# deadskull7/One-Stop-for-COVID-19-Infection-and-Lung-Segmentation-plus-Classification

Hardware: AMD Instinct MI355X
Metric: CT images/sec (fwd+bwd) U-Net 512x512x1 bs16 (higher is better)
Workload: dtype f32 storage / accumulate / parameters; conv products as a two-term fp16 split (3 fp16 MFMAs per multiply, ~2^-22 per product; --algo 2 = strict fp32); 1 GPU; U-Net infection seg (task1 graph T1:853-916), 512x512x1, batch 16/GPU, fp32, fwd+loss+bwd+Keras-Adam; BASELINE.json configs[1]; storage=fp32, global_batch=16, parallelism=dp1, deterministic=False, bn_fold=2

## Files before the change

include/unet_hip.h:

```cpp
#ifndef UNET_HIP_H
#define UNET_HIP_H
#include <stddef.h>
#include <stdint.h>

#ifdef __cplusplus
extern "C" {
#endif

#define UNET_ABI_VERSION 16

typedef struct unet_ctx unet_ctx;
typedef struct unet_model unet_model;
typedef uint16_t unet_bf16;
enum { UNET_DTYPE_F32 = 0, UNET_DTYPE_BF16 = 1 };

enum { UNET_OK = 0, UNET_E_ARG = -1, UNET_E_HIP = -2, UNET_E_SHAPE = -3, UNET_E_STATE = -4, UNET_E_NODEV = -5 };

enum { UNET_ALGO_AUTO = 0, UNET_ALGO_NAIVE = 1, UNET_ALGO_MFMA = 2 };

int32_t unet_abi_version(void);
int32_t unet_ctx_create(int32_t device_id, unet_ctx** out);
void unet_ctx_destroy(unet_ctx* ctx);
const char* unet_last_error(const unet_ctx* ctx);
int32_t unet_ctx_set_profiling(unet_ctx* ctx, int32_t on);
enum { UNET_OPT_RELU_BITS = 1, UNET_OPT_BN_FOLD = 2, UNET_OPT_ENC_BN_FUSED = 3, UNET_OPT_BN_CONCAT_ANALYTIC = 4, UNET_OPT_BN_FUSE_STATS = 5, UNET_OPT_DETERMINISTIC = 6,
       UNET_OPT_HEAD_FUSED = 7, UNET_OPT_SKIP_RAW = 8, UNET_OPT_POOL_SUMS_FUSED = 9, UNET_OPT_HEAD_BWD_FUSED = 10, UNET_OPT_CONV_PP = 13, UNET_OPT_ENC_TAIL_DGRAD = 14,
       UNET_OPT_WGRAD_EARLY_SPLIT = 15 };
int32_t unet_ctx_set_option(unet_ctx* ctx, int32_t option, int32_t value);
int32_t unet_ctx_get_option(unet_ctx* ctx, int32_t option);

enum { UNET_ACT_NONE = 0, UNET_ACT_RELU = 1, UNET_ACT_ELU = 2 };
enum { UNET_MASK_NONE = 0, UNET_MASK_RELU = 1, UNET_MASK_ELU = 2, UNET_MASK_ELU_DROP = 3, UNET_MASK_RELU_BITS = 9  };

size_t unet_conv3x3_w_ws_floats(int32_t cin, int32_t cout);
int32_t unet_conv3x3_pick_algo(int32_t algo, int32_t wd, int32_t cin, int32_t cout);
double unet_conv3x3_exec_ratio(int32_t algo, int32_t h, int32_t wd, int32_t cin, int32_t cout);
double unet_conv3x3_wgrad_exec_ratio(int32_t algo, int32_t h, int32_t wd, int32_t cin, int32_t cout);
int32_t unet_request_bn_stats(unet_ctx*, int32_t c);
int32_t unet_relu_bits_supported(int32_t algo, int32_t h, int32_t wd, int32_t cin, int32_t cout);
size_t unet_relu_bits_bytes(int32_t n, int32_t h, int32_t wd, int32_t c);
int32_t unet_request_relu_bits(unet_ctx*, void* bits);
int32_t unet_allow_k_slices(unet_ctx*);
int32_t unet_ctx_max_kernel_scratch_bytes(unet_ctx*);
int32_t unet_conv3x3_fwd(unet_ctx*, const float* x, const float* w, const float* bias, float* y,
                         int32_t n, int32_t h, int32_t wd, int32_t cin, int32_t cout,
                         int32_t act, float drop_rate, uint64_t drop_seed, int32_t algo, float* w_ws, void* stream);
int32_t unet_conv3x3_fwd_ld(unet_ctx*, const float* x, const float* w, const float* bias, float* y, int32_t ldy,
                            int32_t n, int32_t h, int32_t wd, int32_t cin, int32_t cout, int32_t act, int32_t algo, float* w_ws, void* stream);
int32_t unet_conv3x3_bwd_data(unet_ctx*, const float* dy, const float* w, const float* mask_src,
                              int32_t mask_mode, float mask_rate, uint64_t mask_seed,
// ... 8 lines not shown
                                        int32_t cin, int32_t cout, int32_t algo, void* stream);
int32_t unet_conv3x3_bnfold_bwd_data(unet_ctx*, const float* dy, const float* w, const float* bnp, const double* bn_bwd_sums, double count, const float* x,
                                     int32_t x_channels, int32_t mask_mode, float mask_rate, uint64_t mask_seed, float* dx, float* wt_ws, float* coef,
                                     int32_t n, int32_t h, int32_t wd, int32_t cin, int32_t cout, int32_t algo, void* stream);
int32_t unet_conv3x3_bnfold_bwd_data_enc_tail(unet_ctx*, const float* dy, const float* w, const float* bnp, const double* bn_bwd_sums, double count, const float* x, int32_t ldx,
                                              const float* enc_bnp, const double* enc_sums, double enc_count, const float* skip_k1, const float* dy_pooled, float rate,
                                              uint64_t seed, float* dx, float* wt_ws, float* coef, int32_t n, int32_t h, int32_t wd, int32_t c, int32_t algo, void* stream);
size_t unet_conv3x3_bwd_weights_ws_bytes(int32_t n, int32_t h, int32_t wd, int32_t cin, int32_t cout);
int32_t unet_conv3x3_bwd_weights(unet_ctx*, const float* x, const float* dy, float* dw, float* db,
                                 void* ws, size_t ws_bytes, int32_t n, int32_t h, int32_t wd,
                                 int32_t cin, int32_t cout, int32_t algo, void* stream);

int32_t unet_convT2x2_fwd(unet_ctx*, const float* x, const float* w, const float* bias, float* y,
                          int32_t ldy, int32_t n, int32_t h, int32_t wd, int32_t cin, int32_t cout,
                          int32_t algo, void* stream);
int32_t unet_convT2x2_bwd_data(unet_ctx*, const float* dy, int32_t lddy, const float* w,
                               const float* relu_src, float* dx, int32_t n, int32_t h, int32_t wd,
                               int32_t cin, int32_t cout, int32_t algo, void* stream);
size_t unet_convT2x2_bwd_weights_ws_bytes(int32_t n, int32_t h, int32_t wd, int32_t cin, int32_t cout);
int32_t unet_convT2x2_bwd_weights(unet_ctx*, const float* x, const float* dy, int32_t lddy,
                                  float* dw, float* db, void* ws, size_t ws_bytes, int32_t n,
                                  int32_t h, int32_t wd, int32_t cin, int32_t cout, int32_t algo,
                                  void* stream);

int32_t unet_bn_stats(unet_ctx*, const float* x, int32_t ldx, double* sums, int64_t pixels,
                      int32_t c, void* stream);
int32_t unet_bn_stats_concat(unet_ctx*, const float* x_up, int32_t ldx, const double* src_sums, double src_count, const float* src_gamma,
                             const float* src_beta, double* sums, int64_t pixels, int32_t c_up, int32_t c_skip, void* stream);
int32_t unet_bn_finalize_train(unet_ctx*, const double* sums, double count, const float* gamma,
                               const float* beta, float* moving_mean, float* moving_var,
                               float* bnp, int32_t c, void* stream);
int32_t unet_bn_finalize_infer(unet_ctx*, const float* gamma, const float* beta,
                               const float* moving_mean, const float* moving_var, float* bnp,
                               int32_t c, void* stream);
int32_t unet_bn_apply(unet_ctx*, const float* x, int32_t ldx, const float* bnp, float* y,
                      int32_t ldy, int64_t pixels, int32_t c, void* stream);
int32_t unet_bn_bwd_stats(unet_ctx*, const float* dy, int32_t lddy, const float* x, int32_t ldx,
                          const float* bnp, double* sums, int64_t pixels, int32_t c, void* stream);
int32_t unet_bn_bwd_param_grads(unet_ctx*, const double* sums, float* dgamma, float* dbeta,
                                int32_t c, void* stream);
int32_t unet_bn_bwd_apply(unet_ctx*, const float* dy, int32_t lddy, const float* x, int32_t ldx,
                          const float* bnp, const double* sums, double count, int32_t mask_mode,
                          float mask_rate, uint64_t mask_seed, float* dx, int32_t lddx, int64_t pixels,
                          int32_t c, void* stream);

int32_t unet_maxpool2x2_dropout_fwd(unet_ctx*, const float* x, int32_t ldx, float* y, int32_t n,
// ... 399 lines not shown
```

one-stop-for-covid-19-infection-and-lung-segmentation-plus-classification_amd/_lib.py:

```python
from __future__ import annotations

import ctypes as C
import os

_HERE = os.path.dirname(os.path.abspath(__file__))
LIB_PATH = os.environ.get("COVIDSEG_AMD_LIB") or os.path.join(_HERE, "libunet_hip.so")
ABI_VERSION = 16
COMM_HANDLE_BYTES, COMM_MAX_WORLD, COMM_MAX_DOUBLES = 64, 8, 2048

ALGO_AUTO, ALGO_NAIVE, ALGO_MFMA = 0, 1, 2
OPTIONS = {"relu_bits": 1, "bn_fold": 2, "enc_bn_fused": 3, "bn_concat_analytic": 4, "bn_fuse_stats": 5, "deterministic": 6, "head_fused": 7, "skip_raw": 8, "pool_sums_fused": 9, "head_bwd_fused": 10, "conv_pp": 13, "enc_tail_dgrad": 14, "wgrad_early_split": 15}
ARCH_UNET, ARCH_UNETPP, ARCH_CLASSIFIER = 0, 1, 2
LOSSES = {"bce_dice_loss": 0, "binary_crossentropy": 1, "dice_loss": 2, "tversky_loss": 3, "weighted_bce_dice_loss": 4}
DTYPE_F32, DTYPE_BF16 = 0, 1
ACT_NONE, ACT_RELU, ACT_ELU = 0, 1, 2
MORPH_OPS = {"dilate": 0, "erode": 1, "open": 2, "close": 3}
MORPH_MAX_ITERATIONS = 64
INTENSITY_MAX_EDGES = 63
JOINT_HIST_MAX_K, JOINT_HIST_MAX_BINS = 16, 64
SMOOTH_MAX_RADIUS = 32
PAIRS_CHUNK, PAIRS_LDS_SLOTS = 4096, 1024
PAIRS_MIN_CAPACITY, PAIRS_MAX_CAPACITY = 16, 2 ** 30
TRACK_CLS_NONE, TRACK_CLS_RESOLVED, TRACK_CLS_SHRINKAGE, TRACK_CLS_BOTH, TRACK_CLS_GROWTH, TRACK_CLS_NEW = 0, 1, 2, 3, 4, 5
TEXTURE_MAX_LEVELS, TEXTURE_MAX_DISTANCE, TEXTURE_LDS_COUNTERS = 64, 4, 8192
TEXTURE_MAX_RUN = 2 ** 15
ZONE_MAX_PARTS, ZONE_MAX_SHELLS, ZONE_MAX_BINS = 8, 4, 1024
RANK_MAX_RADIUS = 2
FILTER_MODES = {"nearest": 0, "constant": 1, "reflect": 2}
GEODESIC_MAX_STEP = 65534
MASK_NONE, MASK_RELU, MASK_ELU, MASK_ELU_DROP = 0, 1, 2, 3
PROG_FWD_TRAIN, PROG_BWD, PROG_FWD_INFER = 0, 1, 2
SYNC_BN_FWD, SYNC_LOSS, SYNC_BN_BWD, SYNC_GRAD_BUCKET = 0, 1, 2, 3

f32p = C.POINTER(C.c_float)
# ... 37 lines not shown
    "unet_relu_bits_supported": (i32, [i32, i32, i32, i32, i32]),
    "unet_relu_bits_bytes": (sz, [i32, i32, i32, i32]),
    "unet_request_relu_bits": (i32, [vp, vp]),
    "unet_allow_k_slices": (i32, [vp]),
    "unet_ctx_max_kernel_scratch_bytes": (i32, [vp]),
    "unet_conv3x3_fwd": (i32, [vp, vp, vp, vp, vp, i32, i32, i32, i32, i32, i32, f32, u64, i32, vp, vp]),
    "unet_conv3x3_fwd_ld": (i32, [vp, vp, vp, vp, vp, i32, i32, i32, i32, i32, i32, i32, i32, vp, vp]),
    "unet_conv3x3_bwd_data": (i32, [vp, vp, vp, vp, i32, f32, u64, vp, vp, i32, i32, i32, i32, i32, i32, vp]),
    "unet_conv3x3_bwd_weights_ws_bytes": (sz, [i32, i32, i32, i32, i32]),
    "unet_conv3x3_bwd_weights": (i32, [vp, vp, vp, vp, vp, vp, sz, i32, i32, i32, i32, i32, i32, vp]),
    "unet_convT2x2_fwd": (i32, [vp, vp, vp, vp, vp, i32, i32, i32, i32, i32, i32, i32, vp]),
    "unet_convT2x2_bwd_data": (i32, [vp, vp, i32, vp, vp, vp, i32, i32, i32, i32, i32, i32, vp]),
    "unet_convT2x2_bwd_weights_ws_bytes": (sz, [i32, i32, i32, i32, i32]),
    "unet_convT2x2_bwd_weights": (i32, [vp, vp, vp, i32, vp, vp, vp, sz, i32, i32, i32, i32, i32, i32, vp]),
    "unet_cast_f32_to_bf16": (i32, [vp, vp, vp, i64, vp]),
    "unet_cast_bf16_to_f32": (i32, [vp, vp, vp, i64, vp]),
    "unet_conv3x3_fwd_bf16": (i32, [vp, vp, vp, vp, vp, i32, i32, i32, i32, i32, i32, f32, u64, vp, vp]),
    "unet_conv3x3_first_fwd_bf16": (i32, [vp, vp, vp, vp, vp, i32, i32, i32, i32, i32, f32, u64, vp]),
    "unet_conv3x3_bwd_data_bf16": (i32, [vp, vp, vp, vp, i32, f32, u64, vp, vp, i32, i32, i32, i32, i32, vp]),
    "unet_conv3x3_bwd_weights_ws_bytes_bf16": (sz, [i32, i32, i32, i32, i32]),
    "unet_conv3x3_bwd_weights_bf16": (i32, [vp, vp, vp, vp, vp, vp, sz, i32, i32, i32, i32, i32, vp]),
    "unet_conv3x3_first_bwd_weights_bf16": (i32, [vp, vp, vp, vp, vp, vp, sz, i32, i32, i32, i32, vp]),
    "unet_convT2x2_fwd_bf16": (i32, [vp, vp, vp, vp, vp, i32, i32, i32, i32, i32, i32, vp, vp]),
    "unet_convT2x2_bwd_data_bf16": (i32, [vp, vp, i32, vp, vp, vp, i32, i32, i32, i32, i32, vp, vp]),
    "unet_convT2x2_bwd_weights_ws_bytes_bf16": (sz, [i32, i32, i32, i32, i32]),
    "unet_convT2x2_bwd_weights_bf16": (i32, [vp, vp, vp, i32, vp, vp, vp, sz, i32, i32, i32, i32, i32, vp]),
    "unet_bn_stats": (i32, [vp, vp, i32, vp, i64, i32, vp]),
    "unet_bn_stats_bf16": (i32, [vp, vp, i32, vp, i64, i32, vp]),
    "unet_conv3x3_bnfold_supported": (i32, [i32, i32, i32, i32, i32]),
    "unet_conv3x3_bnfold_ws_floats": (sz, [i32, i32, i32]),
    "unet_conv3x3_bnfold_fwd": (i32, [vp, vp, vp, vp, vp, vp, i32, i32, i32, i32, i32, i32, i32, vp, vp]),
    "unet_conv3x3_bnfold_bwd_weights": (i32, [vp, vp, vp, vp, vp, vp, vp, vp, vp, sz, vp, i32, i32, i32, i32, i32, i32, vp]),
    "unet_conv3x3_bnfold_bwd_data": (i32, [vp, vp, vp, vp, vp, f64, vp, i32, i32, f32, u64, vp, vp, vp, i32, i32, i32, i32, i32, i32, vp]),
    "unet_conv3x3_bnfold_bwd_data_enc_tail": (i32, [vp, vp, vp, vp, vp, f64, vp, i32, vp, vp, f64, vp, vp, f32, u64, vp, vp, vp, i32, i32, i32, i32, i32, vp]),
    "unet_bn_stats_concat": (i32, [vp, vp, i32, vp, f64, vp, vp, vp, i64, i32, i32, vp]),
    "unet_bn_stats_concat_bf16": (i32, [vp, vp, i32, vp, f64, vp, vp, vp, i64, i32, i32, vp]),
    "unet_bn_finalize_train": (i32, [vp, vp, f64, vp, vp, vp, vp, vp, i32, vp]),
    "unet_bn_finalize_infer": (i32, [vp, vp, vp, vp, vp, vp, i32, vp]),
    "unet_bn_apply": (i32, [vp, vp, i32, vp, vp, i32, i64, i32, vp]),
    "unet_bn_apply_bf16": (i32, [vp, vp, i32, vp, vp, i32, i64, i32, vp]),
    "unet_bn_bwd_stats": (i32, [vp, vp, i32, vp, i32, vp, vp, i64, i32, vp]),
    "unet_bn_bwd_stats_bf16": (i32, [vp, vp, i32, vp, i32, vp, vp, i64, i32, vp]),
    "unet_bn_bwd_param_grads": (i32, [vp, vp, vp, vp, i32, vp]),
    "unet_bn_bwd_apply": (i32, [vp, vp, i32, vp, i32, vp, vp, f64, i32, f32, u64, vp, i32, i64, i32, vp]),
    "unet_bn_bwd_apply_bf16": (i32, [vp, vp, i32, vp, i32, vp, vp, f64, i32, f32, u64, vp, i32, i64, i32, vp]),
    "unet_maxpool2x2_dropout_fwd": (i32, [vp, vp, i32, vp, i32, i32, i32, i32, f32, u64, vp]),
# ... 241 lines not shown
```

one-stop-for-covid-19-infection-and-lung-segmentation-plus-classification_amd/csrc/common.h:

```cpp
#pragma once
#include <hip/hip_runtime.h>
#include <stdint.h>
#include <stdio.h>
#include <set>
#include <string>

#include "../../include/unet_hip.h"

constexpr int UNET_BN_SLOTS = 64, UNET_BN_SLOTS_DET = 1024, UNET_BN_SLOT_DOUBLES = 2048;
struct unet_loss_sel { int32_t kind = UNET_LOSS_BCE_DICE; float alpha = 0.5f, beta = 0.5f; };
inline bool unet_loss_sel_ok(const unet_loss_sel& ls, const float* wm = nullptr, bool need_map = true) {
  if (ls.kind < UNET_LOSS_BCE_DICE || ls.kind > UNET_LOSS_WEIGHTED_BCE_DICE) return false;
  if (ls.kind == UNET_LOSS_TVERSKY && !(ls.alpha > 0.0f && ls.beta > 0.0f && ls.alpha < 1e30f && ls.beta < 1e30f)) return false;
  return !need_map || (ls.kind == UNET_LOSS_WEIGHTED_BCE_DICE) == (wm != nullptr);
}
constexpr int UNET_HEAD_SUMS = 100;
struct unet_ctx {
  int device = 0;
  int num_cu = 256;
  int profiling = 0;
  int opt_relu_bits = 1;
  int opt_bn_fold = 2;
  int opt_enc_bn_fused = 1;
  int opt_bn_concat_analytic = 1;
  int opt_bn_fuse_stats = 1;
  int opt_pool_sums_fused = 1;
  int opt_skip_raw = 1;
  int opt_head_fused = 1;
  int opt_head_bwd_fused = 1;
  int opt_enc_tail_dgrad = 1;
  int opt_wgrad_early_split = 0;
  int opt_conv_pp = 1;
  int opt_deterministic = 0;
  double* bn_slots = nullptr;
  int bn_nslots() const { return opt_deterministic ? UNET_BN_SLOTS_DET : UNET_BN_SLOTS; }
  void* convt_img = nullptr;
  size_t convt_img_bytes = 0;
  int k_slices_ok = 0;
  void* splitk_ws = nullptr;
  size_t splitk_ws_bytes = 0;
  int stats_req_c = 0;
  const void* stats_in_slots = nullptr;
  int stats_in_slots_c = 0;
  bool stats_in_slots_xs = false;
  unsigned long long* signs_req = nullptr;
  const void* signs_done = nullptr;
  std::set<const void*> big_lds_kernels;
  std::set<const void*> noted_kernels;
  int max_scratch_bytes = 0;
  std::string err;
};

#define UNET_FAIL(ctx, code, ...)                         \
  do {                                                    \
// ... 326 lines not shown
```

one-stop-for-covid-19-infection-and-lung-segmentation-plus-classification_amd/csrc/model.hip:

```cpp
#include <algorithm>
#include <functional>
#include <map>
#include <set>
#include <string>
#include <vector>

#include "common.h"

extern "C" {

int32_t unet_abi_version(void) { return UNET_ABI_VERSION; }

int32_t unet_ctx_create(int32_t device_id, unet_ctx** out) {
  if (!out) return UNET_E_ARG;
  *out = nullptr;
  int ndev = 0;
  if (hipGetDeviceCount(&ndev) != hipSuccess || ndev <= 0 || device_id < 0 || device_id >= ndev) return UNET_E_NODEV;
  hipDeviceProp_t prop;
  if (hipGetDeviceProperties(&prop, device_id) != hipSuccess) return UNET_E_NODEV;
  if (std::string(prop.gcnArchName).rfind("gfx950", 0) != 0) return UNET_E_NODEV;
  unet_ctx* c = new unet_ctx();
  c->device = device_id;
  c->num_cu = prop.multiProcessorCount;
  const size_t sb = sizeof(double) * UNET_BN_SLOTS_DET * UNET_BN_SLOT_DOUBLES;
// ... 14 lines not shown
  if (ctx && ctx->bn_slots) (void)hipFree(ctx->bn_slots);
  if (ctx && ctx->convt_img) (void)hipFree(ctx->convt_img);
  if (ctx && ctx->splitk_ws) (void)hipFree(ctx->splitk_ws);
  delete ctx;
}
const char* unet_last_error(const unet_ctx* ctx) { return ctx ? ctx->err.c_str() : "null ctx"; }
int32_t unet_ctx_set_profiling(unet_ctx* ctx, int32_t on) { if (!ctx) return UNET_E_ARG; ctx->profiling = on; return UNET_OK; }

static int* ctx_option(unet_ctx* ctx, int32_t option) {
  switch (option) {
    case UNET_OPT_RELU_BITS: return &ctx->opt_relu_bits;
    case UNET_OPT_BN_FOLD: return &ctx->opt_bn_fold;
    case UNET_OPT_ENC_BN_FUSED: return &ctx->opt_enc_bn_fused;
    case UNET_OPT_BN_CONCAT_ANALYTIC: return &ctx->opt_bn_concat_analytic;
    case UNET_OPT_BN_FUSE_STATS: return &ctx->opt_bn_fuse_stats;
    case UNET_OPT_DETERMINISTIC: return &ctx->opt_deterministic;
    case UNET_OPT_HEAD_FUSED: return &ctx->opt_head_fused;
    case UNET_OPT_SKIP_RAW: return &ctx->opt_skip_raw;
    case UNET_OPT_POOL_SUMS_FUSED: return &ctx->opt_pool_sums_fused;
    case UNET_OPT_HEAD_BWD_FUSED: return &ctx->opt_head_bwd_fused;
    case UNET_OPT_CONV_PP: return &ctx->opt_conv_pp;
    case UNET_OPT_ENC_TAIL_DGRAD: return &ctx->opt_enc_tail_dgrad;
    case UNET_OPT_WGRAD_EARLY_SPLIT: return &ctx->opt_wgrad_early_split;
    default: return nullptr;
  }
}
int32_t unet_ctx_set_option(unet_ctx* ctx, int32_t option, int32_t value) {
  if (!ctx) return UNET_E_ARG;
  int* p = ctx_option(ctx, option);
  const int hi = option == UNET_OPT_BN_FOLD ? 3 : (option == UNET_OPT_CONV_PP || option == UNET_OPT_ENC_TAIL_DGRAD) ? 2 : 1;
  if (!p || value < 0 || value > hi) UNET_FAIL(ctx, UNET_E_ARG, "ctx_set_option: option %d value %d", option, value);
  *p = value;
  return UNET_OK;
}
int32_t unet_ctx_get_option(unet_ctx* ctx, int32_t option) {
  if (!ctx) return UNET_E_ARG;
  const int* p = ctx_option(ctx, option);
  if (!p) UNET_FAIL(ctx, UNET_E_ARG, "ctx_get_option: unknown option %d", option);
  return *p;
}

}

static bool use_mfma(int algo, int cin, int cout) {
  if (algo == UNET_ALGO_NAIVE) return false;
  return mfma_conv3x3_supported(cin, cout);
}
static bool use_h2(int algo, int cin, int cout, const void* uws) { return uws && h2_conv3x3_selected(algo, cin, cout); }

static int32_t conv3x3_fwd_dispatch(unet_ctx* ctx, const float* x, const float* w, const float* bias, const float* mask, int mask_mode,
                                    float* y, int n, int h, int wd, int cin, int cout, int act, float rate, uint64_t seed, int algo,
                                    hipStream_t s, float* uws = nullptr, int flip = 0, const float* prepared = nullptr, int ldy = 0) {
  if (ldy && ldy != cout && !(use_h2(algo, cin, cout, uws) && prepared)) UNET_FAIL(ctx, UNET_E_STATE, "conv3x3: a strided output (ldy %d) exists on the h2 kernels with a prepared image only", ldy);
// ... 601 lines not shown
    } else {
      m->grad[nm] = mk(cv, b.n, b.h, b.w, b.c);
    }
  }
  size_t wgb = 0;
  int S2 = m->H, T2 = m->W;
  (void)S2; (void)T2;
  {
    int s = m->H, t = m->W, idx = 0;
    for (auto& l : m->layers) {
      (void)idx;
      if (l.kind != 0) continue;
      int lvl;
      if (l.name == "c5a" || l.name == "c5b") lvl = 4;
      else { int k = l.name[1] - '0'; lvl = (k <= 4) ? k - 1 : 9 - k; }
      int hs = s >> lvl, ts = t >> lvl;
      wgb = std::max(wgb, m->dt ? unet_conv3x3_bwd_weights_ws_bytes_bf16(m->N, hs, ts, l.cin, l.cout) : unet_conv3x3_bwd_weights_ws_bytes(m->N, hs, ts, l.cin, l.cout));
    }
    for (auto& l : m->layers) {
      if (l.kind != 1) continue;
      int k = l.name[1] - '0';
      int lvl = 10 - k;
      wgb = std::max(wgb, m->dt ? bf16_convT_wgrad_ws_bytes(m->N, s >> lvl, t >> lvl, l.cin, l.cout) : unet_convT2x2_bwd_weights_ws_bytes(m->N, s >> lvl, t >> lvl, l.cin, l.cout));
    }
  }
  m->wgrad_ws_bytes = wgb;
  m->off_wgrad_ws = cv.take((wgb + 3) / 4);
  m->ws_floats_train = cv.cur;
}

double nel(const Buf& b) { return (double)b.n * b.h * b.w * b.c; }

#define ADD_OP(vec, nm, fl, by, ...)                          \
  do {                                                        \
    Op _o; _o.name = (nm); _o.flops = (fl); _o.bytes = (by);  \
    _o.run = [=](hipStream_t s) -> int32_t __VA_ARGS__;       \
    (vec).push_back(std::move(_o));                           \
  } while (0)

void arm_bn_statistics(unet_model* m) {
  auto& F = m->prog[UNET_PROG_FWD_TRAIN];
  unet_ctx* ctx = m->ctx;
  for (size_t i = 1; i < F.size(); ++i) {
    if (F[i].name.rfind("bn_stats:", 0) != 0 || F[i - 1].name.rfind("conv3x3_fwd:", 0) != 0) continue;
    const std::string bn = F[i].name.substr(9);
    const auto g = m->tinfo.find(bn + "/gamma");
// ... 402 lines not shown
      const TInfo a = m->tinfo.at(first), b = m->tinfo.at(last_tensor);
      SY.push_back({(int)BW.size() - 1, 3, false, (size_t)a.off * 4, b.off + b.count - a.off});
    };
    if (!dt && m->skip_raw && ctx->opt_enc_bn_fused && ctx->opt_enc_tail_dgrad)
      for (int k = 1; k <= 4; ++k) {
        const std::string bnn = "bn" + std::to_string(k), dca = "c" + std::to_string(10 - k) + "a", cb = "c" + std::to_string(k) + "b";
        const Buf xb = m->act.at(bnn), cg = m->grad.at(cb);
        if (m->fold_c_off.count(dca) && m->skip_k1_off.count(bnn) && m->wprep_b.count(dca) && cg.ld == xb.c && m->act.at(dca).c == xb.c &&
            h2_enc_tail_dgrad_selected(ctx, algo, xb.n, xb.h, xb.w, xb.c, ctx->opt_enc_tail_dgrad == 2))
          m->enc_tail_dgrad.insert(bnn);
      }
    bool enc_split = false;
    const int dec[4] = {256, 128, 64, 32};
    for (int k = 9; k >= 6; --k) {
      int c = dec[k - 6]; std::string ks = std::to_string(k);
      std::string prev = (k == 6) ? "c5b" : "c" + std::to_string(k - 1) + "b";
      int cprev = (k == 6) ? 512 : dec[k - 7];
      conv_bwd("c" + ks + "b", "c" + ks + "a", c, c, true, true, "", m->fold_c_off.count("c" + ks + "a") != 0);
      conv_bwd("c" + ks + "a", "bn" + ks, 2 * c, c, true, false, m->fold_off.count("c" + ks + "a") ? "cat" + ks : "");
      flush_def();
      if (!m->fold_c_off.count("c" + ks + "a")) bn_bwd("bn" + ks, "bn" + ks, "cat" + ks, "cat" + ks, 2 * c, 0, m->fold_off.count("c" + ks + "a") != 0);
      const Buf ib = m->act.at(prev), ug = m->grad.at("u" + ks);
      const std::string un = "u" + ks;
      ADD_OP(BW, "convT_wgrad:" + un, 2.0 * 4 * cprev * c * nel(ib) / ib.c, eb * (nel(ib) + nel(ug)), {
        if (dt) return k_convT_bf16_wgrad(ctx, CBF(m->Av(prev)), CBF(m->Dv(un)), ug.ld, m->G(un + "/kernel"), m->G(un + "/bias"), m->wsf(m->off_wgrad_ws), m->wgrad_ws_bytes, ib.n, ib.h,
                                          ib.w, cprev, c, s);
        return unet_convT2x2_bwd_weights(ctx, m->A(prev), m->D(un), ug.ld, m->G(un + "/kernel"), m->G(un + "/bias"), m->wsf(m->off_wgrad_ws), m->wgrad_ws_bytes,
                                         ib.n, ib.h, ib.w, cprev, c, algo, s);
      });
      ADD_OP(BW, "convT_dgrad:" + un, 2.0 * 4 * cprev * c * nel(ib) / ib.c, eb * (2 * nel(ib) + nel(ug)), {
        if (dt) return k_convT_bf16_dgrad(ctx, CBF(m->Dv(un)), ug.ld, m->P(un + "/kernel"), CBF(m->Av(prev)), WBF(m->Dv(prev)), ib.n, ib.h, ib.w, cprev, c, WBF(static_cast<void*>(m->wsf(m->off_wt))), s);
        const auto so = m->sign_off.find(prev);
        const auto pb = m->wprep_b.find(un);
        const void* img = pb == m->wprep_b.end() ? nullptr : m->wsf(pb->second);
        if (so != m->sign_off.end()) return k_convT_h2_dgrad(ctx, m->D(un), ug.ld, m->P(un + "/kernel"), m->wsf(so->second), m->D(prev), ib.n, ib.h, ib.w, cprev, c, s, 1, img);
        if (img) return k_convT_h2_dgrad(ctx, m->D(un), ug.ld, m->P(un + "/kernel"), m->A(prev), m->D(prev), ib.n, ib.h, ib.w, cprev, c, s, 0, img);
        return unet_convT2x2_bwd_data(ctx, m->D(un), ug.ld, m->P(un + "/kernel"), m->A(prev), m->D(prev), ib.n, ib.h, ib.w, cprev, c, algo, s);
      });
      if (k == 7) bucket("u7/kernel", "out/bias");
      if (k == 6) bucket("u6/kernel", "c6b/bias");
    }
    conv_bwd("c5b", "c5a", 512, 512, true, true);
    conv_bwd("c5a", "p4", 256, 512, true, false, "", ctx->opt_enc_bn_fused != 0);
    if (!ctx->opt_enc_bn_fused) bucket("c5a/kernel", "c5b/bias");
    for (int k = 4; k >= 1; --k) {
      int c = ENC[k - 1]; std::string ks = std::to_string(k);
      const Buf xb = m->act.at("bn" + ks), gb = m->grad.at("bn" + ks);
      const std::string bnn = "bn" + ks, pn = "p" + ks;
      const size_t so = m->bn_bsum_off.at(bnn);
      if (ctx->opt_enc_bn_fused) {
        const std::string dn = "bn" + std::to_string(10 - k), cb = "c" + ks + "b";
        const size_t sod = m->bn_bsum_off.at(dn), bod = m->bnp_off.at(dn), bo = m->bnp_off.at(bnn);
        const Buf cbuf = m->act.at(cb), cg = m->grad.at(cb);
// ... 1008 lines not shown
```

Measured before the change: 1078 images/sec.

## Fuse transposed-conv weight and data gradients into one MFMA kernel

Adds a new HIP kernel that computes the convT2x2 weight gradient and data gradient together in one pass. It loads the upsampled gradient tile into LDS once as split fp16 hi/lo pairs and reuses it for both the wgrad and dgrad MFMAs, applying the ReLU mask inline. The decoder backward graph uses it by default for the shapes it supports (cout 32 or 64). The goal is to avoid reading dU and the activations twice across two kernels and to drop a launch, at the cost of higher register and LDS pressure plus a partial-sum reduction workspace.

```diff
diff --git a/include/unet_hip.h b/include/unet_hip.h
--- a/include/unet_hip.h
+++ b/include/unet_hip.h
@@ -25,7 +25,7 @@
 int32_t unet_ctx_set_profiling(unet_ctx* ctx, int32_t on);
 enum { UNET_OPT_RELU_BITS = 1, UNET_OPT_BN_FOLD = 2, UNET_OPT_ENC_BN_FUSED = 3, UNET_OPT_BN_CONCAT_ANALYTIC = 4, UNET_OPT_BN_FUSE_STATS = 5, UNET_OPT_DETERMINISTIC = 6,
        UNET_OPT_HEAD_FUSED = 7, UNET_OPT_SKIP_RAW = 8, UNET_OPT_POOL_SUMS_FUSED = 9, UNET_OPT_HEAD_BWD_FUSED = 10, UNET_OPT_CONV_PP = 13, UNET_OPT_ENC_TAIL_DGRAD = 14,
-       UNET_OPT_WGRAD_EARLY_SPLIT = 15 };
+       UNET_OPT_WGRAD_EARLY_SPLIT = 15, UNET_OPT_CONVT_BWD_FUSED = 16 };
 int32_t unet_ctx_set_option(unet_ctx* ctx, int32_t option, int32_t value);
 int32_t unet_ctx_get_option(unet_ctx* ctx, int32_t option);
 
@@ -80,6 +80,11 @@
                                   float* dw, float* db, void* ws, size_t ws_bytes, int32_t n,
                                   int32_t h, int32_t wd, int32_t cin, int32_t cout, int32_t algo,
                                   void* stream);
+
+int32_t unet_convT2x2_bwd_fused_selected(unet_ctx*, int32_t n, int32_t h, int32_t wd, int32_t cin, int32_t cout, int32_t force);
+size_t unet_convT2x2_bwd_fused_ws_bytes(int32_t n, int32_t h, int32_t wd, int32_t cin, int32_t cout);
+int32_t unet_convT2x2_bwd_fused(unet_ctx*, const float* x, const float* dy, int32_t lddy, const float* kernel, const void* mask, int32_t mask_is_bits, float* dx, float* dw,
+                                float* db, void* ws, size_t ws_bytes, int32_t n, int32_t h, int32_t wd, int32_t cin, int32_t cout, void* stream);
 
 int32_t unet_bn_stats(unet_ctx*, const float* x, int32_t ldx, double* sums, int64_t pixels,
                       int32_t c, void* stream);
diff --git a/one-stop-for-covid-19-infection-and-lung-segmentation-plus-classification_amd/_lib.py b/one-stop-for-covid-19-infection-and-lung-segmentation-plus-classification_amd/_lib.py
--- a/one-stop-for-covid-19-infection-and-lung-segmentation-plus-classification_amd/_lib.py
+++ b/one-stop-for-covid-19-infection-and-lung-segmentation-plus-classification_amd/_lib.py
@@ -9,7 +9,7 @@
 COMM_HANDLE_BYTES, COMM_MAX_WORLD, COMM_MAX_DOUBLES = 64, 8, 2048
 
 ALGO_AUTO, ALGO_NAIVE, ALGO_MFMA = 0, 1, 2
-OPTIONS = {"relu_bits": 1, "bn_fold": 2, "enc_bn_fused": 3, "bn_concat_analytic": 4, "bn_fuse_stats": 5, "deterministic": 6, "head_fused": 7, "skip_raw": 8, "pool_sums_fused": 9, "head_bwd_fused": 10, "conv_pp": 13, "enc_tail_dgrad": 14, "wgrad_early_split": 15}
+OPTIONS = {"relu_bits": 1, "bn_fold": 2, "enc_bn_fused": 3, "bn_concat_analytic": 4, "bn_fuse_stats": 5, "deterministic": 6, "head_fused": 7, "skip_raw": 8, "pool_sums_fused": 9, "head_bwd_fused": 10, "conv_pp": 13, "enc_tail_dgrad": 14, "wgrad_early_split": 15, "convT_bwd_fused": 16}
 ARCH_UNET, ARCH_UNETPP, ARCH_CLASSIFIER = 0, 1, 2
 LOSSES = {"bce_dice_loss": 0, "binary_crossentropy": 1, "dice_loss": 2, "tversky_loss": 3, "weighted_bce_dice_loss": 4}
 DTYPE_F32, DTYPE_BF16 = 0, 1
@@ -93,6 +93,9 @@
     "unet_conv3x3_bwd_weights_bf16": (i32, [vp, vp, vp, vp, vp, vp, sz, i32, i32, i32, i32, i32, vp]),
     "unet_conv3x3_first_bwd_weights_bf16": (i32, [vp, vp, vp, vp, vp, vp, sz, i32, i32, i32, i32, vp]),
     "unet_convT2x2_fwd_bf16": (i32, [vp, vp, vp, vp, vp, i32, i32, i32, i32, i32, i32, vp, vp]),
+    "unet_convT2x2_bwd_fused_selected": (i32, [vp, i32, i32, i32, i32, i32, i32]),
+    "unet_convT2x2_bwd_fused_ws_bytes": (sz, [i32, i32, i32, i32, i32]),
+    "unet_convT2x2_bwd_fused": (i32, [vp, vp, vp, i32, vp, vp, i32, vp, vp, vp, vp, sz, i32, i32, i32, i32, i32, vp]),
     "unet_convT2x2_bwd_data_bf16": (i32, [vp, vp, i32, vp, vp, vp, i32, i32, i32, i32, i32, vp, vp]),
     "unet_convT2x2_bwd_weights_ws_bytes_bf16": (sz, [i32, i32, i32, i32, i32]),
     "unet_convT2x2_bwd_weights_bf16": (i32, [vp, vp, vp, i32, vp, vp, vp, sz, i32, i32, i32, i32, i32, vp]),
diff --git a/one-stop-for-covid-19-infection-and-lung-segmentation-plus-classification_amd/csrc/common.h b/one-stop-for-covid-19-infection-and-lung-segmentation-plus-classification_amd/csrc/common.h
--- a/one-stop-for-covid-19-infection-and-lung-segmentation-plus-classification_amd/csrc/common.h
+++ b/one-stop-for-covid-19-infection-and-lung-segmentation-plus-classification_amd/csrc/common.h
@@ -30,6 +30,7 @@
   int opt_head_bwd_fused = 1;
   int opt_enc_tail_dgrad = 1;
   int opt_wgrad_early_split = 0;
+  int opt_convT_bwd_fused = 1;
   int opt_conv_pp = 1;
   int opt_deterministic = 0;
   double* bn_slots = nullptr;
diff --git a/one-stop-for-covid-19-infection-and-lung-segmentation-plus-classification_amd/csrc/kernels_convT_bwd.hip b/one-stop-for-covid-19-infection-and-lung-segmentation-plus-classification_amd/csrc/kernels_convT_bwd.hip
--- /dev/null
+++ b/one-stop-for-covid-19-infection-and-lung-segmentation-plus-classification_amd/csrc/kernels_convT_bwd.hip
@@ -0,0 +1,388 @@
+#include <stdlib.h>
+
+#include <algorithm>
+
+#include "common.h"
+
+namespace {
+
+typedef _Float16 f16x8 __attribute__((ext_vector_type(8)));
+typedef short s16x4 __attribute__((ext_vector_type(4)));
+typedef short s16x8 __attribute__((ext_vector_type(8)));
+typedef float f32x4 __attribute__((ext_vector_type(4)));
+typedef unet_f32x16 f32x16;
+
+__device__ __forceinline__ float pow2f(int e) { return __uint_as_float((unsigned)(e + 127) << 23); }
+
+__device__ __forceinline__ f16x8 lds_tr_frag(const char* p0, const char* p1) {
+  typedef __attribute__((address_space(3))) s16x4 lds_s16x4;
+  const s16x4 a = __builtin_amdgcn_ds_read_tr16_b64_v4i16((lds_s16x4*)(p0));
+  const s16x4 b = __builtin_amdgcn_ds_read_tr16_b64_v4i16((lds_s16x4*)(p1));
+  const s16x8 v = __builtin_shufflevector(a, b, 0, 1, 2, 3, 4, 5, 6, 7);
+  return __builtin_bit_cast(f16x8, v);
+}
+
+enum { CTB_MASK_NONE = 0, CTB_MASK_F32 = 1, CTB_MASK_BITS = 2 };
+
+template <int NA>
+__global__ __launch_bounds__(256, 2) void convT_bwd_kernel(const float* __restrict__ A, int ldA, const float* __restrict__ B, const float* __restrict__ Wk, const void* __restrict__ mask,
+                                                           int mask_mode, float* __restrict__ dx, float* __restrict__ part, int N, int H, int W, int CA, int CB, int tiles_b, int strips,
+                                                           int rows_per_chunk, int chunks_per_strip, int nsplit, long long pstride, int units, int upb) {
+  static_assert(NA == 1 || NA == 2, "32 or 64 dU channels");
+  constexpr int R = 1;
+  constexpr int TAPS = 4, AROWS = 2 * R, KP = NA == 1 ? 2 : 1;
+  constexpr int PPL = 32 * 64 + 64, ROWB = 2 * PPL;
+  constexpr int ASUB = AROWS * ROWB, BSUB = R * 32 * 64;
+  constexpr int STAGE1 = NA * ASUB + 2 * BSUB;
+  constexpr int RED = KP > 1 ? 2 * TAPS * 16 * 64 * 4 : 0;
+  constexpr int STAGE = 2 * STAGE1;
+  __shared__ __attribute__((aligned(16))) char smem[STAGE > RED ? STAGE : RED];
+  __shared__ float s_bs[4][64];
+  __shared__ float s_amax[2][4];
+  char* const s_a = smem; char* const s_b = smem + NA * ASUB;
+  const int tid = threadIdx.x, lane = tid & 63, l31 = lane & 31, hi = lane >> 5, l15 = lane & 15, g4 = lane >> 4;
+  const int wave = __builtin_amdgcn_readfirstlane(tid >> 6);
+  const int kp = wave % KP, wb = (wave / KP) % 2, wa = wave / (KP * 2);
+  const int sq = blockIdx.x >> 3;
+  const int tb = sq % tiles_b, split = (sq / tiles_b) * 8 + (blockIdx.x & 7);
+  if (split >= nsplit) return;
+  const int b0 = tb * 64;
+  const int chunk = split % chunks_per_strip; const int ublk = split / chunks_per_strip;
+  const int ya = chunk * rows_per_chunk;
+  const int yb = ya + rows_per_chunk < H ? ya + rows_per_chunk : H;
+  const int HA = 2 * H, WAI = 2 * W;
+
+  f16x8 wfh[TAPS * NA], wfm[TAPS * NA];
+  float unw;
+  {
+    float wv[TAPS * NA][8];
+    float mw = 0.f;
+    const float* wp = Wk + (long long)(g4 * 8) * CB + b0 + wave * 16 + l15;
+#pragma unroll
+    for (int k = 0; k < TAPS * NA; ++k)
+#pragma unroll
+      for (int j = 0; j < 8; ++j) { wv[k][j] = wp[(long long)(k * 32 + j) * CB]; mw = fmaxf(mw, fabsf(wv[k][j])); }
+    mw = wave_max_nonneg(mw);
+    const int ebw = __builtin_amdgcn_readfirstlane((int)((__float_as_uint(mw) >> 23) & 0xFF));
+    const int e_w = ebw >= 11 ? 138 - ebw : 120;
+    const float sw = pow2f(e_w);
+    unw = pow2f(max(-e_w, -126));
+#pragma unroll
+    for (int k = 0; k < TAPS * NA; ++k) {
+      unet_u32x4 h, m;
+#pragma unroll
+      for (int j = 0; j < 4; ++j) { unsigned hh, mm; split2_scaled(wv[k][2 * j], wv[k][2 * j + 1], sw, hh, mm); h[j] = hh; m[j] = mm; }
+      wfh[k] = __builtin_bit_cast(f16x8, h); wfm[k] = __builtin_bit_cast(f16x8, m);
+    }
+  }
+
+  f32x16 acc[TAPS];
+#pragma unroll
+  for (int t = 0; t < TAPS; ++t)
+#pragma unroll
+    for (int r = 0; r < 16; ++r) acc[t][r] = 0.0f;
+  float bsum = 0.0f;
+  int e_a = 120, e_b = 120;
+
+  const int tr_px = (g4 >> 1) * 8 + (l15 >> 2), tr_ch = ((g4 & 1) * 16 + (l15 & 3) * 4) * 2;
+  const char* const pa = s_a + wa * ASUB + tr_ch;
+  const char* const pb = s_b + wb * BSUB + tr_ch;
+  const char* const pd = s_a + l15 * 64 + g4 * 16;
+  const int cq = b0 + wave * 16 + g4 * 4;
+
+  const int u1 = (ublk + 1) * upb < units ? (ublk + 1) * upb : units;
+  for (int unit = ublk * upb; unit < u1; ++unit) {
+    const int cs = unit % strips, n = unit / strips;
+    const int x0 = cs * 32;
+    const __amdgpu_buffer_rsrc_t rs_a = make_rsrc(A + (long long)n * HA * WAI * ldA, (long long)HA * WAI * ldA * 4);
+    const __amdgpu_buffer_rsrc_t rs_b = make_rsrc(B + (long long)n * H * W * CB, (long long)H * W * CB * 4);
+    const int q8 = tid & 7, pc = tid >> 3;
+    int abase_t[NA][2], bbase_t[2];
+#pragma unroll
+    for (int sub = 0; sub < NA; ++sub)
+#pragma unroll
+      for (int half = 0; half < 2; ++half) {
+        const int gx = 2 * x0 + half * 32 + pc;
+        abase_t[sub][half] = gx < WAI ? (gx * ldA + sub * 32 + q8 * 4) * 4 : UNET_OOB;
+      }
+#pragma unroll
+    for (int sub = 0; sub < 2; ++sub) {
+      const int gx = x0 + pc;
+      bbase_t[sub] = gx < W ? (gx * CB + b0 + sub * 32 + q8 * 4) * 4 : UNET_OOB;
+    }
+    constexpr int NAR = NA * AROWS * 2;
+    constexpr int NBR = 2 * R;
+    unet_u32x4 areg[NAR], breg[NBR];
+    auto issue_loads = [&](int ys) __attribute__((always_inline)) {
+#pragma unroll
+      for (int sub = 0; sub < NA; ++sub)
+#pragma unroll
+        for (int row = 0; row < AROWS; ++row)
+#pragma unroll
+          for (int half = 0; half < 2; ++half) {
+            const bool ok = ys + (row >> 1) < yb;
+            areg[(sub * AROWS + row) * 2 + half] = __builtin_amdgcn_raw_buffer_load_b128(rs_a, ok ? abase_t[sub][half] : UNET_OOB, ok ? (2 * ys + row) * WAI * ldA * 4 : 0, 0);
+          }
+#pragma unroll
+      for (int sub = 0; sub < 2; ++sub)
+#pragma unroll
+        for (int row = 0; row < R; ++row) {
+          const bool ok = ys + row < yb;
+          breg[sub * R + row] = __builtin_amdgcn_raw_buffer_load_b128(rs_b, ok ? bbase_t[sub] : UNET_OOB, ok ? (ys + row) * W * CB * 4 : 0, 0);
+        }
+    };
+    auto post_amax = [&]() __attribute__((always_inline)) {
+      float ma = 0.f, mb = 0.f;
+#pragma unroll
+      for (int k = 0; k < NAR; ++k)
+#pragma unroll
+        for (int j = 0; j < 4; ++j) ma = fmaxf(ma, fabsf(__uint_as_float(areg[k][j])));
+#pragma unroll
+      for (int k = 0; k < NBR; ++k)
+#pragma unroll
+        for (int j = 0; j < 4; ++j) mb = fmaxf(mb, fabsf(__uint_as_float(breg[k][j])));
+      ma = wave_max_nonneg(ma); mb = wave_max_nonneg(mb);
+      if (lane == 0) { s_amax[0][wave] = ma; s_amax[1][wave] = mb; }
+    };
+    auto store_lds = [&]() __attribute__((always_inline)) {
+      const float ma = fmaxf(fmaxf(s_amax[0][0], s_amax[0][1]), fmaxf(s_amax[0][2], s_amax[0][3]));
+      const float mb = fmaxf(fmaxf(s_amax[1][0], s_amax[1][1]), fmaxf(s_amax[1][2], s_amax[1][3]));
+      const int eba = __builtin_amdgcn_readfirstlane((int)((__float_as_uint(ma) >> 23) & 0xFF));
+      const int ebb = __builtin_amdgcn_readfirstlane((int)((__float_as_uint(mb) >> 23) & 0xFF));
+      int d = 0;
+      if (eba >= 11 && eba - 127 + e_a >= 15) {
+        const int da_ = 138 - eba - e_a;
+        bsum *= pow2f(max(da_, -126));
+        d += da_; e_a = 138 - eba;
+      }
+      if (ebb >= 11 && ebb - 127 + e_b >= 15) { d += 138 - ebb - e_b; e_b = 138 - ebb; }
+      if (d != 0) {
+        const float f = pow2f(max(d, -126));
+#pragma unroll
+        for (int t = 0; t < TAPS; ++t)
+#pragma unroll
+          for (int r = 0; r < 16; ++r) acc[t][r] *= f;
+      }
+      const float sa = pow2f(e_a), sb = pow2f(e_b);
+      auto put = [&](char* dst, const unet_u32x4& v, float sc) __attribute__((always_inline)) {
+        unsigned h0, m0, h1, m1;
+        split2_scaled(__uint_as_float(v[0]), __uint_as_float(v[1]), sc, h0, m0);
+        split2_scaled(__uint_as_float(v[2]), __uint_as_float(v[3]), sc, h1, m1);
+        *reinterpret_cast<uint2*>(dst) = make_uint2(h0, h1);
+        *reinterpret_cast<uint2*>(dst + STAGE1) = make_uint2(m0, m1);
+      };
+#pragma unroll
+      for (int sub = 0; sub < NA; ++sub)
+#pragma unroll
+        for (int row = 0; row < AROWS; ++row)
+#pragma unroll
+          for (int half = 0; half < 2; ++half) put(s_a + (sub * AROWS + row) * ROWB + (pc & 1) * PPL + (half * 16 + (pc >> 1)) * 64 + q8 * 8, areg[(sub * AROWS + row) * 2 + half], sa);
+#pragma unroll
+      for (int sub = 0; sub < 2; ++sub)
+#pragma unroll
+        for (int row = 0; row < R; ++row) put(s_b + ((sub * R + row) * 32 + pc) * 64 + q8 * 8, breg[sub * R + row], sb);
+    };
+
+    issue_loads(ya);
+    post_amax();
+    __syncthreads();
+    store_lds();
+    __syncthreads();
+    for (int ys = ya; ys < yb; ys += R) {
+      const bool more = ys + R < yb;
+      if (more) issue_loads(ys + R);
+#pragma unroll
+      for (int q = kp; q < 2 * R; q += KP) {
+        const int r = q >> 1, kst = q & 1;
+        const char* bp = pb + (r * 32 + kst * 16 + tr_px) * 64;
+        const f16x8 bh = lds_tr_frag(bp, bp + 4 * 64), bm = lds_tr_frag(bp + STAGE1, bp + STAGE1 + 4 * 64);
+#pragma unroll
+        for (int a = 0; a < 2; ++a) {
+          f16x8 ah[2], am[2];
+#pragma unroll
+          for (int b = 0; b < 2; ++b) {
+            const char* ap = pa + (2 * r + a) * ROWB + b * PPL + (kst * 16 + tr_px) * 64;
+            ah[b] = lds_tr_frag(ap, ap + 4 * 64); am[b] = lds_tr_frag(ap + STAGE1, ap + STAGE1 + 4 * 64);
+            if (wb == 0 && tb == 0) {
+#pragma unroll
+              for (int j = 0; j < 8; ++j) bsum += (float)ah[b][j] + (float)am[b][j];
+            }
+          }
+#pragma unroll
+          for (int b = 0; b < 2; ++b) acc[a * 2 + b] = __builtin_amdgcn_mfma_f32_32x32x16_f16(ah[b], bm, acc[a * 2 + b], 0, 0, 0);
+#pragma unroll
+          for (int b = 0; b < 2; ++b) acc[a * 2 + b] = __builtin_amdgcn_mfma_f32_32x32x16_f16(am[b], bh, acc[a * 2 + b], 0, 0, 0);
+#pragma unroll
+          for (int b = 0; b < 2; ++b) acc[a * 2 + b] = __builtin_amdgcn_mfma_f32_32x32x16_f16(ah[b], bh, acc[a * 2 + b], 0, 0, 0);
+        }
+      }
+#pragma unroll
+      for (int rr = 0; rr < R; ++rr) {
+        const int yr = ys + rr;
+        if (yr >= yb) break;
+        const int px0 = x0 + l15;
+        unsigned mk[2][4];
+        if (mask_mode == CTB_MASK_F32) {
+#pragma unroll
+          for (int t = 0; t < 2; ++t) {
+            const int px = px0 + t * 16;
+            const uint4 v = px < W ? *reinterpret_cast<const uint4*>(static_cast<const float*>(mask) + (((long long)n * H + yr) * W + px) * CB + cq) : make_uint4(0, 0, 0, 0);
+            mk[t][0] = v.x; mk[t][1] = v.y; mk[t][2] = v.z; mk[t][3] = v.w;
+          }
+        } else if (mask_mode == CTB_MASK_BITS) {
+#pragma unroll
+          for (int t = 0; t < 2; ++t) {
+            const int px = px0 + t * 16;
+            const int sh = (px & 7) * 8 + ((cq & 31) >> 2);
+            const unsigned* p = static_cast<const unsigned*>(mask) + (((((long long)n * H + yr) * ((W + 7) >> 3) + (px >> 3)) * (CB >> 5) + (cq >> 5)) * 4) * 2 + (sh >> 5);
+#pragma unroll
+            for (int k = 0; k < 4; ++k) mk[t][k] = px < W ? p[2 * k] : 0u;
+          }
+        }
+        f32x4 dc[2], dh[2];
+#pragma unroll
+        for (int t = 0; t < 2; ++t)
+#pragma unroll
+          for (int r = 0; r < 4; ++r) { dc[t][r] = 0.f; dh[t][r] = 0.f; }
+#pragma unroll
+        for (int k = 0; k < TAPS * NA; ++k) {
+          const int ab = k / NA, sub = k % NA;
+          const char* p = pd + (sub * AROWS + 2 * rr + (ab >> 1)) * ROWB + (ab & 1) * PPL;
+          f16x8 uh[2], um[2];
+#pragma unroll
+          for (int t = 0; t < 2; ++t) { uh[t] = *reinterpret_cast<const f16x8*>(p + t * 16 * 64); um[t] = *reinterpret_cast<const f16x8*>(p + t * 16 * 64 + STAGE1); }
+#pragma unroll
+          for (int t = 0; t < 2; ++t) dc[t] = __builtin_amdgcn_mfma_f32_16x16x32_f16(wfh[k], um[t], dc[t], 0, 0, 0);
+#pragma unroll
+          for (int t = 0; t < 2; ++t) dh[t] = __builtin_amdgcn_mfma_f32_16x16x32_f16(wfh[k], uh[t], dh[t], 0, 0, 0);
+#pragma unroll
+          for (int t = 0; t < 2; ++t) dc[t] = __builtin_amdgcn_mfma_f32_16x16x32_f16(wfm[k], uh[t], dc[t], 0, 0, 0);
+        }
+        {
+          const float un = pow2f(max(-e_a, -126)) * unw;
+#pragma unroll
+          for (int t = 0; t < 2; ++t) {
+            const int px = px0 + t * 16;
+            float v[4];
+#pragma unroll
+            for (int r = 0; r < 4; ++r) v[r] = (dc[t][r] + dh[t][r]) * un;
+            if (mask_mode == CTB_MASK_F32) {
+#pragma unroll
+              for (int r = 0; r < 4; ++r) v[r] = __uint_as_float(mk[t][r]) > 0.0f ? v[r] : 0.0f;
+            } else if (mask_mode == CTB_MASK_BITS) {
+              const int sh = ((px & 7) * 8 + ((cq & 31) >> 2)) & 31;
+#pragma unroll
+              for (int r = 0; r < 4; ++r) v[r] = ((mk[t][r] >> sh) & 1u) ? v[r] : 0.0f;
+            }
+            if (px < W) {
+              float* q = dx + (((long long)n * H + yr) * W + px) * CB + cq;
+              __builtin_nontemporal_store(v[0], q); __builtin_nontemporal_store(v[1], q + 1); __builtin_nontemporal_store(v[2], q + 2); __builtin_nontemporal_store(v[3], q + 3);
+            }
+          }
+        }
+      }
+      if (more) post_amax();
+      __syncthreads();
+      if (more) { store_lds(); __syncthreads(); }
+    }
+  }
+  const float un_a = pow2f(max(-e_a, -126));
+  const float un = un_a * pow2f(max(-e_b, -126));
+#pragma unroll
+  for (int t = 0; t < TAPS; ++t)
+#pragma unroll
+    for (int r = 0; r < 16; ++r) acc[t][r] *= un;
+  bsum *= un_a;
+
+  bsum += __shfl_xor(bsum, 32, 64);
+  if (KP > 1) {
+    float* red = reinterpret_cast<float*>(smem);
+    float* img = red + (size_t)wb * (TAPS * 16 * 64);
+    s_bs[wave][lane] = bsum;
+    if (kp == 1) {
+#pragma unroll
+      for (int t = 0; t < TAPS; ++t)
+#pragma unroll
+        for (int r = 0; r < 16; ++r) img[(t * 16 + r) * 64 + lane] = acc[t][r];
+    }
+    __syncthreads();
+    if (kp == 0) {
+#pragma unroll
+      for (int t = 0; t < TAPS; ++t)
+#pragma unroll
+        for (int r = 0; r < 16; ++r) acc[t][r] += img[(t * 16 + r) * 64 + lane];
+      bsum = s_bs[wave][lane] + s_bs[wave + 1][lane];
+    }
+  }
+  if (kp != 0) return;
+  float* P = part + (long long)split * pstride;
+  const int ar = wa * 32, bc = b0 + wb * 32 + l31;
+#pragma unroll
+  for (int t = 0; t < TAPS; ++t)
+#pragma unroll
+    for (int r = 0; r < 16; ++r) {
+      const int m = (r & 3) + 8 * (r >> 2) + 4 * hi;
+      P[((long long)t * CA + ar + m) * CB + bc] = acc[t][r];
+    }
+  if (wb == 0 && tb == 0 && lane < 32) P[(long long)TAPS * CA * CB + ar + l31] = bsum;
+}
+
+struct CtbPlan { int tiles_b, strips, rows_per_chunk, chunks_per_strip, nsplit, units, upb; size_t floats; };
+
+CtbPlan plan_ctb(int n, int h, int w, int cin, int cout) {
+  CtbPlan p;
+  p.tiles_b = cin / 64; p.strips = (w + 31) / 32;
+  const long long per = 4LL * cout * cin, units = (long long)n * p.strips;
+  long long want = std::max<long long>(1, 512 / p.tiles_b);
+  want = std::min(want, std::max<long long>(1, (64LL << 20) / per));
+  p.units = (int)units; p.upb = (int)std::max<long long>(1, units / want);
+  const long long ublocks = (units + p.upb - 1) / p.upb;
+  long long cps = std::max<long long>(1, want / ublocks);
+  cps = std::min<long long>(cps, std::max<long long>(1, h / 4));
+  p.rows_per_chunk = (int)((h + cps - 1) / cps); p.chunks_per_strip = (h + p.rows_per_chunk - 1) / p.rows_per_chunk;
+  p.nsplit = (int)(ublocks * p.chunks_per_strip);
+  p.floats = (size_t)p.nsplit * (per + cout) + wgrad_reduce_scratch_floats(4, cout, cin, cout, p.nsplit);
+  return p;
+}
+
+bool ctb_supported(int n, int h, int wd, int cin, int cout) {
+  return n >= 1 && h >= 1 && wd >= 1 && (cout == 32 || cout == 64) && cin >= 64 && (cin % 64) == 0;
+}
+
+}
+
+extern "C" {
+
+int32_t unet_convT2x2_bwd_fused_selected(unet_ctx* ctx, int32_t n, int32_t h, int32_t wd, int32_t cin, int32_t cout, int32_t force) {
+  if (!ctx || !ctb_supported(n, h, wd, cin, cout)) return 0;
+  if (16LL * h * wd * cout >= (1LL << 30) || 4LL * h * wd * cin >= (1LL << 30)) return 0;
+  if (force) return 1;
+  return (long long)n * ((wd + 31) / 32) * std::max(1, h / 4) * (cin / 64) >= 2LL * ctx->num_cu ? 1 : 0;
+}
+
+size_t unet_convT2x2_bwd_fused_ws_bytes(int32_t n, int32_t h, int32_t wd, int32_t cin, int32_t cout) {
+  return ctb_supported(n, h, wd, cin, cout) ? plan_ctb(n, h, wd, cin, cout).floats * sizeof(float) : 0;
+}
+
+int32_t unet_convT2x2_bwd_fused(unet_ctx* ctx, const float* x, const float* dy, int32_t lddy, const float* kernel, const void* mask, int32_t mask_is_bits, float* dx, float* dw, float* db,
+                                void* ws, size_t ws_bytes, int32_t n, int32_t h, int32_t wd, int32_t cin, int32_t cout, void* stream) {
+  if (!ctx || !x || !dy || !kernel || !dx || !dw || !db || lddy < cout || (lddy & 3)) UNET_FAIL(ctx, UNET_E_ARG, "convT_bwd_fused: bad args");
+  if (!ctb_supported(n, h, wd, cin, cout)) UNET_FAIL(ctx, UNET_E_SHAPE, "convT_bwd_fused: cin=%d cout=%d unsupported (cout 32 or 64, cin a multiple of 64)", cin, cout);
+  if (4LL * h * wd * lddy * 4 >= (1LL << 30) || (long long)h * wd * cin * 4 >= (1LL << 30)) UNET_FAIL(ctx, UNET_E_SHAPE, "convT_bwd_fused: one image must stay below 1 GiB (32-bit buffer offsets)");
+  const CtbPlan p = plan_ctb(n, h, wd, cin, cout);
+  if (!ws || ws_bytes < p.floats * sizeof(float)) UNET_FAIL(ctx, UNET_E_ARG, "convT_bwd_fused: workspace %zu < %zu bytes", ws_bytes, p.floats * sizeof(float));
+  float* part = static_cast<float*>(ws);
+  const long long S = 4LL * cout * cin + cout;
+  const int mm = mask ? (mask_is_bits ? CTB_MASK_BITS : CTB_MASK_F32) : CTB_MASK_NONE;
+  const dim3 grid((unsigned)(8 * ((p.nsplit + 7) / 8) * p.tiles_b));
+  hipStream_t s = as_stream(stream);
+#define UNET_CTB(NA_) do { auto kern = convT_bwd_kernel<NA_>; unet_note_kernel(ctx, reinterpret_cast<const void*>(kern)); \
+    hipLaunchKernelGGL(kern, grid, dim3(256), 0, s, dy, lddy, x, kernel, mask, mm, dx, part, n, h, wd, cout, cin, p.tiles_b, p.strips, p.rows_per_chunk, p.chunks_per_strip, p.nsplit, S, \
+                       p.units, p.upb); } while (0)
+  if (cout == 64) UNET_CTB(2); else UNET_CTB(1);
+#undef UNET_CTB
+  UNET_CHECK_LAUNCH(ctx, "convT_bwd_fused");
+  return k_wgrad_reduce(ctx, part, p.nsplit, 4, cout, cin, cout, dw, db, s);
+}
+
+}
diff --git a/one-stop-for-covid-19-infection-and-lung-segmentation-plus-classification_amd/csrc/model.hip b/one-stop-for-covid-19-infection-and-lung-segmentation-plus-classification_amd/csrc/model.hip
--- a/one-stop-for-covid-19-infection-and-lung-segmentation-plus-classification_amd/csrc/model.hip
+++ b/one-stop-for-covid-19-infection-and-lung-segmentation-plus-classification_amd/csrc/model.hip
@@ -60,13 +60,14 @@
     case UNET_OPT_CONV_PP: return &ctx->opt_conv_pp;
     case UNET_OPT_ENC_TAIL_DGRAD: return &ctx->opt_enc_tail_dgrad;
     case UNET_OPT_WGRAD_EARLY_SPLIT: return &ctx->opt_wgrad_early_split;
+    case UNET_OPT_CONVT_BWD_FUSED: return &ctx->opt_convT_bwd_fused;
     default: return nullptr;
   }
 }
 int32_t unet_ctx_set_option(unet_ctx* ctx, int32_t option, int32_t value) {
   if (!ctx) return UNET_E_ARG;
   int* p = ctx_option(ctx, option);
-  const int hi = option == UNET_OPT_BN_FOLD ? 3 : (option == UNET_OPT_CONV_PP || option == UNET_OPT_ENC_TAIL_DGRAD) ? 2 : 1;
+  const int hi = option == UNET_OPT_BN_FOLD ? 3 : (option == UNET_OPT_CONV_PP || option == UNET_OPT_ENC_TAIL_DGRAD || option == UNET_OPT_CONVT_BWD_FUSED) ? 2 : 1;
   if (!p || value < 0 || value > hi) UNET_FAIL(ctx, UNET_E_ARG, "ctx_set_option: option %d value %d", option, value);
   *p = value;
   return UNET_OK;
@@ -714,6 +715,7 @@
       int k = l.name[1] - '0';
       int lvl = 10 - k;
       wgb = std::max(wgb, m->dt ? bf16_convT_wgrad_ws_bytes(m->N, s >> lvl, t >> lvl, l.cin, l.cout) : unet_convT2x2_bwd_weights_ws_bytes(m->N, s >> lvl, t >> lvl, l.cin, l.cout));
+      if (!m->dt && m->ctx->opt_convT_bwd_fused) wgb = std::max(wgb, unet_convT2x2_bwd_fused_ws_bytes(m->N, s >> lvl, t >> lvl, l.cin, l.cout));
     }
   }
   m->wgrad_ws_bytes = wgb;
@@ -1162,13 +1164,22 @@
       if (!m->fold_c_off.count("c" + ks + "a")) bn_bwd("bn" + ks, "bn" + ks, "cat" + ks, "cat" + ks, 2 * c, 0, m->fold_off.count("c" + ks + "a") != 0);
       const Buf ib = m->act.at(prev), ug = m->grad.at("u" + ks);
       const std::string un = "u" + ks;
-      ADD_OP(BW, "convT_wgrad:" + un, 2.0 * 4 * cprev * c * nel(ib) / ib.c, eb * (nel(ib) + nel(ug)), {
+      const bool ct_fused = !dt && algo == UNET_ALGO_AUTO && ctx->opt_convT_bwd_fused &&
+                            unet_convT2x2_bwd_fused_selected(ctx, ib.n, ib.h, ib.w, cprev, c, ctx->opt_convT_bwd_fused == 2) &&
+                            m->wgrad_ws_bytes >= unet_convT2x2_bwd_fused_ws_bytes(ib.n, ib.h, ib.w, cprev, c);
+      if (ct_fused) ADD_OP(BW, "convT_bwd:" + un, 2.0 * 2.0 * 4 * cprev * c * nel(ib) / ib.c, eb * (2 * nel(ib) + nel(ug)), {
+        const auto so = m->sign_off.find(prev);
+        const bool bits = so != m->sign_off.end();
+        return unet_convT2x2_bwd_fused(ctx, m->A(prev), m->D(un), ug.ld, m->P(un + "/kernel"), bits ? static_cast<const void*>(m->wsf(so->second)) : static_cast<const void*>(m->A(prev)), bits ? 1 : 0,
+                                       m->D(prev), m->G(un + "/kernel"), m->G(un + "/bias"), m->wsf(m->off_wgrad_ws), m->wgrad_ws_bytes, ib.n, ib.h, ib.w, cprev, c, s);
+      });
+      if (!ct_fused) ADD_OP(BW, "convT_wgrad:" + un, 2.0 * 4 * cprev * c * nel(ib) / ib.c, eb * (nel(ib) + nel(ug)), {
         if (dt) return k_convT_bf16_wgrad(ctx, CBF(m->Av(prev)), CBF(m->Dv(un)), ug.ld, m->G(un + "/kernel"), m->G(un + "/bias"), m->wsf(m->off_wgrad_ws), m->wgrad_ws_bytes, ib.n, ib.h,
                                           ib.w, cprev, c, s);
         return unet_convT2x2_bwd_weights(ctx, m->A(prev), m->D(un), ug.ld, m->G(un + "/kernel"), m->G(un + "/bias"), m->wsf(m->off_wgrad_ws), m->wgrad_ws_bytes,
                                          ib.n, ib.h, ib.w, cprev, c, algo, s);
       });
-      ADD_OP(BW, "convT_dgrad:" + un, 2.0 * 4 * cprev * c * nel(ib) / ib.c, eb * (2 * nel(ib) + nel(ug)), {
+      if (!ct_fused) ADD_OP(BW, "convT_dgrad:" + un, 2.0 * 4 * cprev * c * nel(ib) / ib.c, eb * (2 * nel(ib) + nel(ug)), {
         if (dt) return k_convT_bf16_dgrad(ctx, CBF(m->Dv(un)), ug.ld, m->P(un + "/kernel"), CBF(m->Av(prev)), WBF(m->Dv(prev)), ib.n, ib.h, ib.w, cprev, c, WBF(static_cast<void*>(m->wsf(m->off_wt))), s);
         const auto so = m->sign_off.find(prev);
         const auto pb = m->wprep_b.find(un);
```

New measurement: 1086 images/sec, median of 6. About the same (+0.7%).
